# ubc-vision/COTR

Measured on NVIDIA H100. Metric: query-points/sec (256x256 pair, 1024 queries), higher is better.
Workload: dtype f32 (fp16 hi/lo split operands, fp32 accumulate on wgmma)

## Files before the change

cotr_b200/csrc/common.cuh:

```cuda
#pragma once
#include <cuda_fp16.h>
#include <cuda_runtime.h>
#include <cstdarg>
#include <cstdint>
#include <cstdio>

namespace cotr {

void set_error(const char* fmt, ...);

#define COTR_CHECK_CUDA(expr)                                                                      \
    do {                                                                                           \
        cudaError_t e_ = (expr);                                                                   \
        if (e_ != cudaSuccess) {                                                                   \
            ::cotr::set_error("%s:%d: %s -> %s", __FILE__, __LINE__, #expr, cudaGetErrorString(e_)); \
            return 1;                                                                              \
        }                                                                                          \
    } while (0)

#define COTR_CHECK(cond, ...)                                                                      \
    do {                                                                                           \
        if (!(cond)) {                                                                             \
            ::cotr::set_error(__VA_ARGS__);                                                        \
            return 1;                                                                              \
// ... 27 lines not shown
    attr[0].id = cudaLaunchAttributeProgrammaticStreamSerialization;
    attr[0].val.programmaticStreamSerializationAllowed = 1;
    cfg.attrs = attr;
    cfg.numAttrs = g_use_pdl ? 1 : 0;
    return cudaLaunchKernelEx(&cfg, kernel, KArgs(args)...);
}

template <typename... KArgs, typename... Args>
inline cudaError_t launch_kernel_cluster(void (*kernel)(KArgs...), dim3 grid, dim3 block, size_t smem, cudaStream_t s,
                                         int cluster_z, Args... args) {
    cudaLaunchConfig_t cfg = {};
    cfg.gridDim = grid;
    cfg.blockDim = block;
    cfg.dynamicSmemBytes = smem;
    cfg.stream = s;
    cudaLaunchAttribute attr[2];
    int n = 0;
    if (g_use_pdl) {
        attr[n].id = cudaLaunchAttributeProgrammaticStreamSerialization;
        attr[n].val.programmaticStreamSerializationAllowed = 1;
        ++n;
    }
    if (cluster_z > 1) {
        attr[n].id = cudaLaunchAttributeClusterDimension;
        attr[n].val.clusterDim.x = 1;
        attr[n].val.clusterDim.y = 1;
        attr[n].val.clusterDim.z = (unsigned)cluster_z;
        ++n;
    }
    cfg.attrs = attr;
    cfg.numAttrs = n;
    return cudaLaunchKernelEx(&cfg, kernel, KArgs(args)...);
}

constexpr int kNumSms = 132;

constexpr int kDModel = 256;
constexpr int kHeads = 8;
constexpr int kHeadDim = 32;
constexpr int kTokens = 512;
constexpr int kFF = 1024;
constexpr int kEncLayers = 6;
constexpr int kDecLayers = 6;

constexpr size_t kAttnKPlaneBytes = 4 * 512 * 16;
constexpr size_t kAttnKImgBytes = 2 * kAttnKPlaneBytes;
constexpr size_t kAttnVGroupBytes = 2 * 32 * 16 + 16;
constexpr size_t kAttnVImgBytes = 64 * kAttnVGroupBytes;
constexpr size_t kAttnHeadImgBytes = kAttnKImgBytes + kAttnVImgBytes;

struct Split16 {
    __half* hi;
    __half* lo;
};
struct CSplit16 {
    const __half* hi;
    const __half* lo;
};
inline CSplit16 cs(const Split16& s) { return CSplit16{s.hi, s.lo}; }
inline Split16 offset(const Split16& s, size_t elems) { return Split16{s.hi + elems, s.lo + elems}; }
inline CSplit16 offset(const CSplit16& s, size_t elems) { return CSplit16{s.hi + elems, s.lo + elems}; }

constexpr int kStemCanvasRows = 262, kStemCanvasPitch = 264;
constexpr size_t kStemCanvasElems = (size_t)kStemCanvasRows * kStemCanvasPitch * 4;
constexpr int kStemK = 7 * 32;

// ... 122 lines not shown
```

cotr_b200/csrc/gemm_tc.cu:

```cuda
#include <cmath>
#include <cstring>
#include <vector>

#include "a_loader.cuh"
#include "tc_common.cuh"

namespace cotr {

int g_tc_variant = 0;
int g_use_pdl = 1;

namespace {

using namespace tc;

constexpr int BK = 64;
constexpr int kThreads = 384;
constexpr int kConsumerThreads = 256;
constexpr int kBarConsumers = 6;
constexpr long long kWaveCtas = 144;

enum LoaderMode : int { LD_GATHER = 0, LD_CONV = 1, LD_STEM4 = 2 };

__host__ __device__ inline int tc_npad(int N) { return N >= 64 ? ((N + 63) / 64) * 64 : ((N + 15) / 16) * 16; }

template <int BN>
struct Cfg {
    static constexpr int BM = BN >= 256 ? 64 : 128;
    static constexpr int WN = BN >= 256 ? 128 : BN;
    static constexpr uint32_t kAPlane = BM * 128u;
    static constexpr uint32_t kBPlane = BN * 128u;
    static constexpr uint32_t kStage = 2 * kAPlane + 2 * kBPlane;
    static constexpr int kStagesRaw = (int)((227u * 1024u - 3072u) / kStage);
    static constexpr int kStages = kStagesRaw > 4 ? 4 : kStagesRaw;
    static constexpr int kMain = WN >= 128 ? 1 : (WN == 64 ? 2 : 4);
    static constexpr int kCorr = WN >= 64 ? 1 : 2;
    static constexpr int kAccRegs = WN / 2;
    static constexpr uint32_t kAccPitch = BN * 4u + 16u;
    static constexpr uint32_t kAccTileBytes = ((BM * kAccPitch + 1023u) / 1024u) * 1024u;
    static constexpr uint32_t kOutPitch = BN * 2u + 16u;
    static constexpr uint32_t kWarpStaging = 2u * 32u * kOutPitch;
    static constexpr int kChunksN = BN / 16;
    static constexpr int kEpiHalves = (BN >= 32 && BN < 256) ? 2 : 1;
    static constexpr int kChunksW = kChunksN / kEpiHalves;
    static constexpr int kRing = kChunksW < 2 ? kChunksW : 2;
    static constexpr uint32_t kVecOffset = kStages * kStage + 256;
    static constexpr uint32_t kVecBytes = 2u * BN * 4u + 2u * BM * 8u;
    static constexpr uint32_t kSmemBytes = kStages * kStage + 2048 + kVecBytes;
    static constexpr uint32_t kPartOffset = kVecOffset + kVecBytes;
    static constexpr uint32_t kPartPitch = BN * 4u;
    static constexpr int kMaxSplit = BN <= 64 ? 4 : 1;
    static constexpr uint32_t kPartMaxBytes = kMaxSplit > 1 ? 96u * kPartPitch : 0u;
    static_assert(kSmemBytes + kPartMaxBytes <= 227u * 1024u, "split-K partial tiles do not fit");
    static_assert(kStages >= 2, "pipeline needs at least two stages");
    static_assert(kAccTileBytes + (BM / 32) * kWarpStaging <= kStages * kStage, "epilogue tiles do not fit the idle stages");
    static_assert(kStage % 1024 == 0 && kAPlane % 1024 == 0, "stages must stay 1024-byte aligned for SWIZZLE_128B");
    static_assert(kMaxSplit == 1 || BM == 128, "split-K hands over 32-row groups of a 128-row tile");
};

struct EpiOperands {
    float4 bias[4];
    float4 add[4];
    uint4 res_hi[2], res_lo[2];
};

template <int BN, bool LN, int MODE, bool DLN>
__global__ void __launch_bounds__(kThreads, 1) gemm_tc_kernel(const GemmParams p, const int npad) {
    using C = Cfg<BN>;
    constexpr int BM = C::BM;
    extern __shared__ uint8_t smem_raw[];
    const uint32_t raw_addr = smem_u32(smem_raw);
    uint8_t* stage_base = smem_raw + (((raw_addr + 1023u) & ~1023u) - raw_addr);
    uint64_t* bars = reinterpret_cast<uint64_t*>(stage_base + C::kStages * C::kStage);
    uint64_t* full_a = bars;
    uint64_t* empty = bars + C::kStages;
    uint64_t* part_full = bars + 2 * C::kStages;
    uint64_t* vec_full = bars + 2 * C::kStages + 1;
    float* vec_a = reinterpret_cast<float*>(stage_base + C::kVecOffset);
    float* vec_b = vec_a + BN;
    float2* st_a = reinterpret_cast<float2*>(vec_b + BN);
    float2* st_r = st_a + BM;
    float* acc_tile = reinterpret_cast<float*>(stage_base);
    static_assert(!DLN || (MODE == LD_GATHER && !LN), "deferred LayerNorm: row-major operand tiles only");
    constexpr bool kCanLnA = DLN;
    const bool has_aln = kCanLnA && p.a_ln_cs != nullptr;
    const bool stage_vec = kCanLnA && !LN && (has_aln || p.res_ln_part != nullptr);

    const int warp = threadIdx.x >> 5, lane = threadIdx.x & 31;
    const int m0 = blockIdx.x * BM;
    const int n0 = blockIdx.y * BN;
    const int ksplit = gridDim.z;
    const int kz = blockIdx.z;
    const int KC = ((p.K + BK - 1) / BK) / ksplit;
    const int it0 = kz * KC;

    if (threadIdx.x == 0) {
        for (int s = 0; s < C::kStages; ++s) {
            mbar_init(&full_a[s], 129);
            mbar_init(&empty[s], 8);
        }
        mbar_init(part_full, 1);
        if (DLN) mbar_init(vec_full, 64);
        mbar_fence_init();
        if (ksplit > 1) mbar_arrive_expect_tx(part_full, (uint32_t)(ksplit - 1) * (uint32_t)(BM / ksplit) * C::kPartPitch);
    }
    __syncthreads();
    if (ksplit > 1) cluster_arrive();

    if (warp >= 8) {
        const int t = threadIdx.x - kConsumerThreads;
        const int kg = t & 7;
        const int rb = t >> 3;
        constexpr int kRowIters = BM / 16;
        const uint8_t* wimg = reinterpret_cast<const uint8_t*>(p.Wtc);
        auto load_weights = [&](int it) {
            const int s = it % C::kStages;
            mbar_arrive_expect_tx(&full_a[s], 2u * C::kBPlane);
            uint8_t* b_dst = stage_base + (size_t)s * C::kStage + 2 * C::kAPlane;
            const uint8_t* src = wimg + (((size_t)(it0 + it) * 2) * npad + n0) * 128;
            tma_bulk_g2s(b_dst, src, C::kBPlane, &full_a[s]);
            tma_bulk_g2s(b_dst + C::kBPlane, src + (size_t)npad * 128, C::kBPlane, &full_a[s]);
        };
        const int u = (warp - 10) * 32 + lane;
        const float* src_a = has_aln ? p.a_ln_cs : p.res_ln_gamma;
        float va[(BN + 63) / 64], vb[(BN + 63) / 64];
        if (stage_vec && warp >= 10) {
#pragma unroll
            for (int k = 0; k < (BN + 63) / 64; ++k) {
                const int i = u + 64 * k;
                const bool ok = i < BN && n0 + i < p.N;
                va[k] = ok ? __ldg(src_a + n0 + i) : 0.f;
                vb[k] = (ok && !has_aln) ? __ldg(p.res_ln_beta + n0 + i) : 0.f;
            }
        }
        ARow rows[kRowIters];
#pragma unroll
        for (int i = 0; i < kRowIters; ++i) rows[i] = decode_a_row(p, m0 + rb + 16 * i);
        const uint32_t a_off = (uint32_t)rb * 128u + (uint32_t)((kg ^ (rb & 7)) << 4);
        const uint32_t dst0 = smem_u32(stage_base) + a_off;
        if (t == 0) {
            for (int it = 0; it < KC && it < C::kStages; ++it) load_weights(it);
            pdl_launch_dependents();
        }
        pdl_wait();

#pragma unroll 1
        for (int it = 0; it < KC; ++it) {
            const int s = it % C::kStages;
            const uint32_t ph = (uint32_t)(it / C::kStages) & 1u;
            mbar_wait(&empty[s], ph ^ 1u);
            if (t == 0 && it >= C::kStages) load_weights(it);
            const int k0 = (it0 + it) * BK;
            {
                const uint32_t dst = dst0 + (uint32_t)s * C::kStage;
                int kh = 0, kw = 0, koff = k0 + kg * 8;
                if constexpr (MODE == LD_CONV) {
                    const int tap = k0 / p.C;
                    koff = k0 - tap * p.C + kg * 8;
                    kh = tap / p.KW;
                    kw = tap - kh * p.KW;
                }
                if constexpr (MODE == LD_STEM4) {
                    const int kk = k0 + kg * 8;
                    koff = (kk >> 5) * (kStemCanvasPitch * 4) + (kk & 31);
                }
                const bool k_ok = (k0 + kg * 8) < p.K;
#pragma unroll
                for (int i = 0; i < kRowIters; ++i) {
                    bool ok = rows[i].valid && k_ok;
                    size_t off = rows[i].off + koff;
                    if constexpr (MODE == LD_CONV) {
                        const int ih = rows[i].ih0 + kh, iw = rows[i].iw0 + kw;
                        ok = ok && ih >= 0 && ih < p.H && iw >= 0 && iw < p.W;
                        off = rows[i].off + ((size_t)ih * p.W + iw) * p.C + koff;
                    }
                    if (!ok) off = 0;
                    const uint32_t bytes = ok ? 16u : 0u;
                    cp_async16(dst + i * 2048, p.a.hi + off, bytes);
                    cp_async16(dst + C::kAPlane + i * 2048, p.a.lo + off, bytes);
                }
                cp_async_mbar_arrive_noinc(&full_a[s]);
            }
        }

// ... 29 lines not shown
            for (int k = 0; k < (BN + 63) / 64; ++k) {
                const int i = u + 64 * k;
                if (i < BN) { vec_a[i] = va[k]; vec_b[i] = vb[k]; }
            }
            if (has_aln) stage_stats(p.a_ln_part, st_a);
            if (p.res_ln_part != nullptr) stage_stats(p.res_ln_part, st_r);
            mbar_arrive(vec_full);
        }
    } else {
        const int wg = warp >> 2;
        const uint32_t a_sub = BN >= 256 ? 0u : (uint32_t)wg * 64u * 128u;
        const uint32_t b_sub = BN >= 256 ? (uint32_t)wg * 128u * 128u : 0u;
        float acc_m[C::kMain][C::kAccRegs], acc_c[C::kCorr][C::kAccRegs];
#pragma unroll
        for (int a = 0; a < C::kMain; ++a)
#pragma unroll
            for (int j = 0; j < C::kAccRegs; ++j) acc_m[a][j] = 0.f;
#pragma unroll
        for (int a = 0; a < C::kCorr; ++a)
#pragma unroll
            for (int j = 0; j < C::kAccRegs; ++j) acc_c[a][j] = 0.f;
        auto mma = [&](float (&d)[C::kAccRegs], uint64_t da, uint64_t db) {
            if constexpr (C::WN == 16) wgmma_ss_n16(d, da, db);
            else if constexpr (C::WN == 32) wgmma_ss_n32(d, da, db);
            else if constexpr (C::WN == 64) wgmma_ss_n64(d, da, db);
            else wgmma_ss_n128(d, da, db);
        };
        auto fence_all = [&]() {
#pragma unroll
            for (int a = 0; a < C::kMain; ++a) fence_regs(acc_m[a]);
#pragma unroll
            for (int a = 0; a < C::kCorr; ++a) fence_regs(acc_c[a]);
        };
#pragma unroll 1
        for (int it = 0; it < KC; ++it) {
            const int s = it % C::kStages;
            const uint32_t ph = (uint32_t)(it / C::kStages) & 1u;
            mbar_wait(&full_a[s], ph);
            fence_proxy_async_smem();
            const uint32_t a_addr = smem_u32(stage_base + (size_t)s * C::kStage);
            const uint32_t b_addr = a_addr + 2 * C::kAPlane;
            fence_all();
            wgmma_fence();
#pragma unroll
            for (int ks = 0; ks < BK / 16; ++ks) {
                const uint64_t dah = make_desc_sw128(a_addr + a_sub + 32 * ks);
                const uint64_t dal = make_desc_sw128(a_addr + C::kAPlane + a_sub + 32 * ks);
                const uint64_t dbh = make_desc_sw128(b_addr + b_sub + 32 * ks);
                const uint64_t dbl = make_desc_sw128(b_addr + C::kBPlane + b_sub + 32 * ks);
                mma(acc_c[0], dal, dbh);
                mma(acc_m[ks % C::kMain], dah, dbh);
                mma(acc_c[C::kCorr - 1], dah, dbl);
            }
            wgmma_commit();
            wgmma_wait<1>();
            fence_all();
            if (it > 0 && lane == 0) mbar_arrive(&empty[(it - 1) % C::kStages]);
        }
        wgmma_wait<0>();
        fence_all();
        named_barrier_sync(kBarConsumers, kConsumerThreads);
        const int r0 = (BN >= 256 ? 0 : wg * 64) + (warp & 3) * 16 + (lane >> 2);
        const int c0 = (BN >= 256 ? wg * 128 : 0) + 2 * (lane & 3);
#pragma unroll
        for (int j = 0; j < C::kAccRegs; j += 2) {
            float v[2];
#pragma unroll
            for (int e = 0; e < 2; ++e) {
                float x = acc_c[0][j + e];
#pragma unroll
                for (int a = 1; a < C::kCorr; ++a) x += acc_c[a][j + e];
                float y = acc_m[0][j + e];
#pragma unroll
                for (int a = 1; a < C::kMain; ++a) y += acc_m[a][j + e];
                v[e] = x + y;
            }
            const int row = r0 + ((j >> 1) & 1) * 8;
            const int col = c0 + (j >> 2) * 8;
            *reinterpret_cast<float2*>(reinterpret_cast<uint8_t*>(acc_tile) + (uint32_t)row * C::kAccPitch + col * 4) = make_float2(v[0], v[1]);
        }
        named_barrier_sync(kBarConsumers, kConsumerThreads);
    }

    const int ew = warp & 3;
    const int half = warp >> 2;
    if (ksplit > 1) cluster_wait();
    if (warp < 8 && half < C::kEpiHalves && ew * 32 < BM) {
        pdl_wait();
        const int cbeg = half * C::kChunksW * 16;
        const int row = m0 + ew * 32 + lane;
        const int owner = (ew * ksplit) >> 2;
        const bool mine = owner == kz;
        const bool row_ok = mine && row < p.M;
        uint8_t* arow = reinterpret_cast<uint8_t*>(acc_tile) + (uint32_t)(ew * 32 + lane) * C::kAccPitch;
        const float* add_row = (row_ok && p.addmat) ? p.addmat + (size_t)(row % p.add_period) * p.ld_add : nullptr;
        const bool has_res = row_ok && p.res.hi != nullptr;
        const size_t res_off = (size_t)(row_ok ? row : 0) * p.ldr;
        const float acc_scale = p.acc_scale;
        const bool res_ln = kCanLnA && has_res && p.res_ln_part != nullptr;
        float2 res_st = make_float2(0.f, 1.f);
        float res_shift = 0.f;
        float2 a_st = make_float2(0.f, 1.f);
        const bool emit_part = kCanLnA && row_ok && p.ln_part_out != nullptr;
        const bool tail = p.out_f32 != nullptr && (p.N & 15) != 0;
        const bool has_bias = p.bias != nullptr && !tail;

        auto prefetch = [&](int nb, EpiOperands& o) {
            if (nb >= p.N || tail) return;
// ... 53 lines not shown
        constexpr uint32_t kPartPitch = C::kPartPitch, kPartOffset = C::kPartOffset;
        const uint32_t part_slot = (uint32_t)(BM / ksplit) * kPartPitch;
        const uint32_t part_row = (uint32_t)((ew - owner * (4 / ksplit)) * 32 + lane) * kPartPitch;
        const uint32_t part_swz = (uint32_t)(lane & 7);
        auto sum_acc = [&](int c, float (&v)[16]) {
#pragma unroll
            for (int j = 0; j < 16; j += 4) {
                const float4 t4 = *reinterpret_cast<const float4*>(arow + (c + j) * 4);
                v[j] = t4.x; v[j + 1] = t4.y; v[j + 2] = t4.z; v[j + 3] = t4.w;
            }
        };
        auto finish_acc = [&](int c, float (&v)[16]) {
            if (ksplit > 1) {
                const uint8_t* part = stage_base + kPartOffset + part_row;
                for (int peer = 0; peer < ksplit - 1; ++peer) {
#pragma unroll
                    for (int j = 0; j < 16; j += 4) {
                        const uint32_t piece = ((uint32_t)((c + j) >> 2) ^ part_swz) << 4;
                        const float4 t4 = *reinterpret_cast<const float4*>(part + (uint32_t)peer * part_slot + piece);
                        v[j] += t4.x; v[j + 1] += t4.y; v[j + 2] += t4.z; v[j + 3] += t4.w;
                    }
                }
            }
#pragma unroll
            for (int j = 0; j < 16; ++j) v[j] *= acc_scale;
        };
        auto load_acc = [&](int c, float (&v)[16]) {
            sum_acc(c, v);
            finish_acc(c, v);
        };

        size_t tile_base = 0;
        const bool direct = p.out_f32 != nullptr || out_location(p, m0, n0, tile_base);
        uint8_t* const stg_base = stage_base + C::kAccTileBytes;
        uint8_t* stg = stg_base + (uint32_t)ew * C::kWarpStaging + (uint32_t)lane * C::kOutPitch;
        auto emit16 = [&](int c, const float (&v)[16]) {
            if (direct) {
                if (row_ok && n0 + c < p.N) store16(p, row, n0 + c, v);
                return;
            }
            uint4 h0, l0, h1, l1;
            split_f16x2(v[0], v[1], h0.x, l0.x);   split_f16x2(v[2], v[3], h0.y, l0.y);
            split_f16x2(v[4], v[5], h0.z, l0.z);   split_f16x2(v[6], v[7], h0.w, l0.w);
            split_f16x2(v[8], v[9], h1.x, l1.x);   split_f16x2(v[10], v[11], h1.y, l1.y);
            split_f16x2(v[12], v[13], h1.z, l1.z); split_f16x2(v[14], v[15], h1.w, l1.w);
            uint8_t* d = stg + c * 2;
            *reinterpret_cast<uint4*>(d) = h0;
            *reinterpret_cast<uint4*>(d + 16) = h1;
            *reinterpret_cast<uint4*>(d + 32 * C::kOutPitch) = l0;
            *reinterpret_cast<uint4*>(d + 32 * C::kOutPitch + 16) = l1;
        };
        auto drain_plane = [&](int plane) {
            constexpr int kLanesPerRow = BN * 2 / 16;
            constexpr int kRowsPerPass = kLanesPerRow >= 32 ? 1 : 32 / kLanesPerRow;
            constexpr int kPiecesPerLane = kLanesPerRow > 32 ? kLanesPerRow / 32 : 1;
            const uint8_t* wbase = stg_base + (uint32_t)ew * C::kWarpStaging;
            const int r_in = kLanesPerRow >= 32 ? 0 : lane / kLanesPerRow;
            const int piece0 = kLanesPerRow >= 32 ? lane : lane % kLanesPerRow;
            __half* gout = (plane == 0 ? p.out.hi : p.out.lo) + tile_base;
#pragma unroll 4
            for (int r0 = 0; r0 < 32; r0 += kRowsPerPass) {
                const int rr = r0 + r_in;
                const int grow_ = m0 + ew * 32 + rr;
#pragma unroll
                for (int q = 0; q < kPiecesPerLane; ++q) {
                    const int piece = piece0 + q * 32;
                    const uint4 val = *reinterpret_cast<const uint4*>(wbase + (uint32_t)(plane * 32 + rr) * C::kOutPitch + piece * 16);
                    if (grow_ < p.M)
                        *reinterpret_cast<uint4*>(gout + (size_t)(ew * 32 + rr) * p.ldc + piece * 8) = val;
                }
            }
        };
        auto drain = [&]() {
            if (direct) return;
            if constexpr (C::kEpiHalves == 2) {
                named_barrier_sync(1 + ew, 64);
                drain_plane(half);
            } else {
                __syncwarp();
                drain_plane(0);
                drain_plane(1);
            }
        };

        EpiOperands ops[C::kRing];
        const int nbase = (LN ? 0 : n0) + cbeg;
#pragma unroll
        for (int i = 0; i < C::kRing; ++i) prefetch(nbase + 16 * i, ops[i]);
        if (kCanLnA && (has_aln || p.res_ln_part != nullptr)) {
            mbar_wait(vec_full, 0);
            if (has_aln) a_st = st_a[ew * 32 + lane];
            if (res_ln) { res_st = st_r[ew * 32 + lane]; res_shift = -res_st.x * res_st.y; }
        }
        constexpr bool kPreload = !LN && C::kChunksW <= 2;
        float pre[kPreload ? C::kChunksW : 1][16];
        if constexpr (kPreload) {
#pragma unroll
            for (int ci = 0; ci < C::kChunksW; ++ci) sum_acc(cbeg + ci * 16, pre[ci]);
        }
        if (C::kMaxSplit > 1 && ksplit > 1) {
            if (!mine) {
                const uint32_t local = smem_u32(stage_base) + kPartOffset + (uint32_t)(kz < owner ? kz : kz - 1) * part_slot + part_row;
// ... 74 lines not shown
            const float mean = sum * (1.f / 256.f);
            const float dm = mean - shift;
            const float var = fmaxf(sq * (1.f / 256.f) - dm * dm, 0.f);
            const float rstd = 1.f / sqrtf(var + 1e-5f);
#pragma unroll 1
            for (int c = 0; c < BN; c += 32) {
#pragma unroll
                for (int h = 0; h < 2; ++h) {
                    float r[16];
                    sum_acc(c + h * 16, r);
                    float v[16];
#pragma unroll
                    for (int j = 0; j < 16; j += 4) {
                        const float4 g4 = __ldg(reinterpret_cast<const float4*>(p.ln_gamma + c + h * 16 + j));
                        const float4 b4 = __ldg(reinterpret_cast<const float4*>(p.ln_beta + c + h * 16 + j));
                        v[j] = (r[j] - mean) * rstd * g4.x + b4.x;
                        v[j + 1] = (r[j + 1] - mean) * rstd * g4.y + b4.y;
                        v[j + 2] = (r[j + 2] - mean) * rstd * g4.z + b4.z;
                        v[j + 3] = (r[j + 3] - mean) * rstd * g4.w + b4.w;
                    }
                    emit16(c + h * 16, v);
                }
            }
            drain();
        }
        }
    }

    __syncthreads();
}

template <int BN, bool LN, int MODE, bool DLN = false>
int launch_one(const GemmParams& p, cudaStream_t s) {
    using C = Cfg<BN>;
    static unsigned long long configured = 0;
    if (first_use_on_device(&configured)) {
        COTR_CHECK_CUDA(cudaFuncSetAttribute(gemm_tc_kernel<BN, LN, MODE, DLN>, cudaFuncAttributeMaxDynamicSharedMemorySize,
                                             (int)(C::kSmemBytes + C::kPartMaxBytes)));
    }
    const int npad = tc_npad(p.N);
    dim3 grid((p.M + C::BM - 1) / C::BM, (p.N + BN - 1) / BN);
    int ksplit = 1;
    if constexpr (!LN && BN <= 64 && MODE != LD_STEM4) {
        const int kc = (p.K + BK - 1) / BK;
        const long long ctas = (long long)grid.x * grid.y;
        if (!(g_tc_variant & 512) && kc >= (16 >> ((g_tc_variant >> 14) & 3))) {
            if (C::kMaxSplit >= 4 && kc % 4 == 0 && ctas * 4 <= kWaveCtas) ksplit = 4;
            else if (C::kMaxSplit >= 2 && kc % 2 == 0 && ctas * 2 <= kWaveCtas) ksplit = 2;
        }
    }
    COTR_CHECK(p.a_ln_cs == nullptr || (DLN && p.K == 256 && p.a_mode == A_ROWMAJOR && p.a_ln_part != nullptr),
               "gemm_tc: the deferred LayerNorm on A needs a row-major operand with K = 256 and its partial statistics");
    COTR_CHECK((p.res_ln_part == nullptr && p.ln_part_out == nullptr) || DLN,
               "gemm_tc: deferred-LayerNorm residual / statistics on an unsupported tile");
    COTR_CHECK(p.ln_part_out == nullptr || (p.N == 256 && !p.remap && p.out_f32 == nullptr), "gemm_tc: row statistics need a plain N = 256 output");
    grid.z = ksplit;
    const size_t smem = C::kSmemBytes + (size_t)(ksplit - 1) * (C::BM / ksplit) * C::kPartPitch;
    COTR_CHECK_CUDA(launch_kernel_cluster(gemm_tc_kernel<BN, LN, MODE, DLN>, grid, dim3(kThreads), smem, s, ksplit, p, npad));
    return 0;
}

template <int BN, bool LN>
int launch_mode(const GemmParams& p, cudaStream_t s) {
    const bool gather = (p.a_mode == A_ROWMAJOR || p.a_mode == A_TOKENS);
    if (gather && (p.K & 7) == 0 && (p.lda & 7) == 0) {
        if constexpr (!LN) {
            const bool dln = p.a_ln_cs != nullptr || p.res_ln_part != nullptr || p.ln_part_out != nullptr;
            if (dln) return launch_one<BN, LN, LD_GATHER, true>(p, s);
        }
        return launch_one<BN, LN, LD_GATHER>(p, s);
    }
    if constexpr (!LN && BN >= 32) {
        if (p.a_mode == A_CONV_NHWC && (p.C & 63) == 0) return launch_one<BN, LN, LD_CONV>(p, s);
    }
    if constexpr (!LN && BN == 64) {
        if (p.a_mode == A_STEM_NHWC4 && p.K == kStemK) return launch_one<64, false, LD_STEM4>(p, s);
    }
    set_error("gemm_tc: no kernel instantiation for a_mode %d, K %d, lda %d, C %d with tile N %d", p.a_mode, p.K, p.lda, p.C, BN);
    return 1;
}

inline uint16_t f32_to_f16_rn(float f) {
    uint32_t x;
    memcpy(&x, &f, 4);
    const uint16_t sign = (uint16_t)((x >> 16) & 0x8000u);
    x &= 0x7FFFFFFFu;
    if (x >= 0x47800000u) return sign | 0x7BFFu;
    if (x < 0x38800000u) {
        float af;
        memcpy(&af, &x, 4);
        const uint32_t m = (uint32_t)nearbyintf(af * 16777216.0f);
        return sign | (uint16_t)m;
    }
    const uint32_t mant = x & 0x7FFFFFu;
    uint32_t h = (((x >> 23) - 112u) << 10) | (mant >> 13);
    const uint32_t rem = mant & 0x1FFFu;
    if (rem > 0x1000u || (rem == 0x1000u && (h & 1u))) ++h;
    if (h >= 0x7C00u) h = 0x7BFFu;
    return sign | (uint16_t)h;
}
inline float f16_to_f32(uint16_t h) {
    const uint32_t sign = (uint32_t)(h & 0x8000u) << 16;
    const uint32_t e = (h >> 10) & 0x1Fu, m = h & 0x3FFu;
    float mag;
    if (e == 0) mag = (float)m * (1.0f / 16777216.0f);
    else {
// ... 29 lines not shown
    const float scale = ldexpf(1.f, e);
    uint16_t* out = reinterpret_cast<uint16_t*>(dst_host);
    for (int kc = 0; kc < kc_n; ++kc)
        for (int r = 0; r < npad; ++r)
            for (int c = 0; c < 8; ++c)
                for (int el = 0; el < 8; ++el) {
                    const int k = kc * BK + c * 8 + el;
                    const float x = (r < N && k < K) ? w[(size_t)r * K + k] * scale : 0.f;
                    const uint16_t hi = f32_to_f16_rn(x);
                    const uint16_t lo = f32_to_f16_rn(x - f16_to_f32(hi));
                    const size_t pos = (size_t)r * 64 + (size_t)((c ^ (r & 7)) * 8) + el;
                    out[((size_t)kc * 2 + 0) * npad * 64 + pos] = hi;
                    out[((size_t)kc * 2 + 1) * npad * 64 + pos] = lo;
                }
    return ldexpf(1.f, -e);
}

int launch_gemm_tc(const GemmParams& p, cudaStream_t s) {
    COTR_CHECK(p.M > 0 && p.N > 0 && p.K > 0, "gemm_tc: empty problem %d x %d x %d", p.M, p.N, p.K);
    COTR_CHECK(p.Wtc != nullptr, "gemm_tc: weight has no tensor-core image");
    COTR_CHECK(p.out_f32 != nullptr || (p.N & 15) == 0, "gemm_tc: split16 outputs need N %% 16 == 0 (N=%d)", p.N);
    COTR_CHECK(p.res.hi == nullptr || ((p.ldr & 15) == 0 && (p.N & 15) == 0 && ((uintptr_t)p.res.hi & 31) == 0 && ((uintptr_t)p.res.lo & 31) == 0),
               "gemm_tc: residual needs ldr %% 16 == 0 and 32-byte aligned planes");
    COTR_CHECK(p.addmat == nullptr || ((p.ld_add & 3) == 0 && (p.N & 15) == 0), "gemm_tc: add-matrix needs ld %% 4 == 0");
    COTR_CHECK(p.out_f32 != nullptr || (p.ldc & 7) == 0, "gemm_tc: split16 output needs ldc %% 8 == 0");
    if (p.ln_gamma) {
        COTR_CHECK(p.N == 256 && p.relu == 0 && p.out_f32 == nullptr && !p.remap, "gemm_tc: LayerNorm epilogue needs N = 256");
        return launch_mode<256, true>(p, s);
    }
    if (p.N < 64) {
        COTR_CHECK(p.N <= 16, "gemm_tc: N between 17 and 63 is not instantiated");
        return launch_mode<16, false>(p, s);
    }
    const long long mt = (p.M + 127) / 128;
    static const long long kThr[4] = {86, 43, 57, 132};
    const long long thr64 = kThr[(g_tc_variant >> 10) & 3];
    if (mt * ((p.N + 63) / 64) >= thr64 || p.a_mode == A_STEM_NHWC4 || (p.N % 32) != 0) return launch_mode<64, false>(p, s);
    return launch_mode<32, false>(p, s);
}

}
```

cotr_b200/csrc/mlp_tc.cu:

```cuda
#include "split16.cuh"
#include "tc_common.cuh"

namespace cotr {

namespace {

using namespace tc;

constexpr int BM = 64;
constexpr int BK = 64;
constexpr int kThreads = 384;
constexpr int kConsumerThreads = 256;
constexpr int kBarConsumers = 6;
constexpr int kK1Chunks = kDModel / BK;

template <int S>
struct MlpCfg {
    static constexpr int HS = kFF / S;
    static constexpr int WN1 = HS / 2;
    static constexpr int kMain1 = WN1 >= 128 ? 1 : 2;
    static constexpr int kK2Chunks = HS / BK;
    static constexpr int kIters = kK1Chunks + kK2Chunks;
    static constexpr uint32_t kAPlane = BM * 128u;
    static constexpr uint32_t kW1Plane = HS * 128u;
// ... 233 lines not shown
            pdl_wait();
            float v[8];
            const uint8_t* own = base + (uint32_t)rr * C::kAccPitch + lane * 32;
            const float4 a0 = *reinterpret_cast<const float4*>(own), a1 = *reinterpret_cast<const float4*>(own + 16);
            v[0] = a0.x; v[1] = a0.y; v[2] = a0.z; v[3] = a0.w; v[4] = a1.x; v[5] = a1.y; v[6] = a1.z; v[7] = a1.w;
#pragma unroll 1
            for (int slot = 0; slot < S - 1; ++slot) {
                const uint8_t* pp = base + C::kPartOffset + (uint32_t)(slot * C::kOwnRows + w) * C::kRowBytes + lane * 32;
                const float4 b0 = *reinterpret_cast<const float4*>(pp), b1 = *reinterpret_cast<const float4*>(pp + 16);
                v[0] += b0.x; v[1] += b0.y; v[2] += b0.z; v[3] += b0.w; v[4] += b1.x; v[5] += b1.y; v[6] += b1.z; v[7] += b1.w;
            }
            float bias[8], res[8];
            load_vec8(p.b2, lane, bias);
            const size_t off = (size_t)row * kDModel + lane * 8;
            load8_split(p.x, off, res);
#pragma unroll
            for (int j = 0; j < 8; ++j) v[j] = v[j] * p.w2_scale + bias[j] + res[j];
            warp_layernorm256(v, p.g, p.be, lane);
            if (p.g2) warp_layernorm256(v, p.g2, p.be2, lane);
            store8_split(p.out, off, v);
        }
    }
}

template <int S>
int configure(size_t* smem) {
    static unsigned long long configured = 0;
    *smem = MlpCfg<S>::kSmemBytes;
    if (first_use_on_device(&configured))
        COTR_CHECK_CUDA(cudaFuncSetAttribute(mlp_tc_kernel<S>, cudaFuncAttributeMaxDynamicSharedMemorySize, (int)MlpCfg<S>::kSmemBytes));
    return 0;
}

int max_clusters_of_8(int* out) {
    static int cached[64] = {0};
    int dev = 0;
    cudaGetDevice(&dev);
    if (cached[dev & 63] > 0) { *out = cached[dev & 63]; return 0; }
    size_t smem = 0;
    if (configure<8>(&smem)) return 1;
    cudaLaunchConfig_t cfg = {};
    cfg.gridDim = dim3(1, 1, 8);
    cfg.blockDim = dim3(kThreads);
    cfg.dynamicSmemBytes = smem;
    cudaLaunchAttribute attr[1];
    attr[0].id = cudaLaunchAttributeClusterDimension;
    attr[0].val.clusterDim.x = 1;
    attr[0].val.clusterDim.y = 1;
    attr[0].val.clusterDim.z = 8;
    cfg.attrs = attr;
    cfg.numAttrs = 1;
    int n = 0;
    COTR_CHECK_CUDA(cudaOccupancyMaxActiveClusters(&n, mlp_tc_kernel<8>, &cfg));
    cached[dev & 63] = n;
    *out = n;
    return 0;
}

template <int S>
int launch_split(const MlpParams& p, cudaStream_t s) {
    size_t smem = 0;
    if (configure<S>(&smem)) return 1;
    const dim3 grid((p.M + BM - 1) / BM, 1, S);
    COTR_CHECK_CUDA(launch_kernel_cluster(mlp_tc_kernel<S>, grid, dim3(kThreads), smem, s, S, p));
    return 0;
}

}

int launch_mlp_tc(const MlpParams& p, cudaStream_t s) {
    COTR_CHECK(p.M > 0 && p.w1 && p.w2 && p.b1 && p.b2 && p.g && p.be && (p.g2 == nullptr) == (p.be2 == nullptr),
               "mlp_tc: bad parameters (M %d)", p.M);
    const int tiles = (p.M + BM - 1) / BM;
    int n8 = 0;
    if (max_clusters_of_8(&n8)) return 1;
    if (tiles <= n8) return launch_split<8>(p, s);
    return launch_split<4>(p, s);
}

}
```

Before: 1.013 million.

## Pick split-K by cluster occupancy and fold extra K segments in shared memory

Replaces the fixed 144-CTA wave limit for choosing split-K with a query of cudaOccupancyMaxActiveClusters, and factors that query into a shared helper also used by the MLP launcher. For small-N tiles (BN<=32), when a smaller split than the largest divisor is chosen, each CTA now periodically folds its wgmma accumulators into a per-thread shared-memory buffer at segment boundaries. This keeps the per-segment accumulation the same as a full split while using fewer CTAs. It adds extra wgmma_wait<0> drains and shared-memory traffic inside the K loop, and it raises the shared-memory requirement for these tiles.

```diff
diff --git a/cotr_b200/csrc/common.cuh b/cotr_b200/csrc/common.cuh
--- a/cotr_b200/csrc/common.cuh
+++ b/cotr_b200/csrc/common.cuh
@@ -83,6 +83,8 @@
     cfg.numAttrs = n;
     return cudaLaunchKernelEx(&cfg, kernel, KArgs(args)...);
 }
+
+int max_active_clusters(const void* kernel, int threads, size_t smem, int cluster, int* cache, int* out);
 
 constexpr int kNumSms = 132;
 
diff --git a/cotr_b200/csrc/gemm_tc.cu b/cotr_b200/csrc/gemm_tc.cu
--- a/cotr_b200/csrc/gemm_tc.cu
+++ b/cotr_b200/csrc/gemm_tc.cu
@@ -9,6 +9,31 @@
 
 int g_tc_variant = 0;
 int g_use_pdl = 1;
+
+int max_active_clusters(const void* kernel, int threads, size_t smem, int cluster, int* cache, int* out) {
+    int dev = 0;
+    COTR_CHECK_CUDA(cudaGetDevice(&dev));
+    if (cache[dev & 63] > 0) {
+        *out = cache[dev & 63];
+        return 0;
+    }
+    cudaLaunchConfig_t cfg = {};
+    cfg.gridDim = dim3(1, 1, cluster);
+    cfg.blockDim = dim3(threads);
+    cfg.dynamicSmemBytes = smem;
+    cudaLaunchAttribute attr[1];
+    attr[0].id = cudaLaunchAttributeClusterDimension;
+    attr[0].val.clusterDim.x = 1;
+    attr[0].val.clusterDim.y = 1;
+    attr[0].val.clusterDim.z = (unsigned)cluster;
+    cfg.attrs = attr;
+    cfg.numAttrs = 1;
+    int n = 0;
+    COTR_CHECK_CUDA(cudaOccupancyMaxActiveClusters(&n, kernel, &cfg));
+    cache[dev & 63] = n;
+    *out = n;
+    return 0;
+}
 
 namespace {
 
@@ -18,7 +43,6 @@
 constexpr int kThreads = 384;
 constexpr int kConsumerThreads = 256;
 constexpr int kBarConsumers = 6;
-constexpr long long kWaveCtas = 144;
 
 enum LoaderMode : int { LD_GATHER = 0, LD_CONV = 1, LD_STEM4 = 2 };
 
@@ -51,7 +75,10 @@
     static constexpr uint32_t kPartPitch = BN * 4u;
     static constexpr int kMaxSplit = BN <= 64 ? 4 : 1;
     static constexpr uint32_t kPartMaxBytes = kMaxSplit > 1 ? 96u * kPartPitch : 0u;
-    static_assert(kSmemBytes + kPartMaxBytes <= 227u * 1024u, "split-K partial tiles do not fit");
+    static constexpr bool kFold = kMaxSplit > 1 && BN <= 32;
+    static constexpr uint32_t kFoldOffset = kPartOffset + kPartMaxBytes;
+    static constexpr uint32_t kFoldBytes = kFold ? (uint32_t)kConsumerThreads * kAccRegs * 4u : 0u;
+    static_assert(kSmemBytes + kPartMaxBytes + kFoldBytes <= 227u * 1024u, "split-K partial tiles do not fit");
     static_assert(kStages >= 2, "pipeline needs at least two stages");
     static_assert(kAccTileBytes + (BM / 32) * kWarpStaging <= kStages * kStage, "epilogue tiles do not fit the idle stages");
     static_assert(kStage % 1024 == 0 && kAPlane % 1024 == 0, "stages must stay 1024-byte aligned for SWIZZLE_128B");
@@ -65,7 +92,7 @@
 };
 
 template <int BN, bool LN, int MODE, bool DLN>
-__global__ void __launch_bounds__(kThreads, 1) gemm_tc_kernel(const GemmParams p, const int npad) {
+__global__ void __launch_bounds__(kThreads, 1) gemm_tc_kernel(const GemmParams p, const int npad, const int seg) {
     using C = Cfg<BN>;
     constexpr int BM = C::BM;
     extern __shared__ uint8_t smem_raw[];
@@ -245,6 +272,18 @@
 #pragma unroll
             for (int a = 0; a < C::kCorr; ++a) fence_regs(acc_c[a]);
         };
+        auto acc_sum = [&](int j) {
+            float x = acc_c[0][j];
+#pragma unroll
+            for (int a = 1; a < C::kCorr; ++a) x += acc_c[a][j];
+            float y = acc_m[0][j];
+#pragma unroll
+            for (int a = 1; a < C::kMain; ++a) y += acc_m[a][j];
+            return x + y;
+        };
+        float* fold = reinterpret_cast<float*>(stage_base + C::kFoldOffset) + threadIdx.x;
+        const bool folding = C::kFold && seg < KC;
+        int fold_next = seg;
 #pragma unroll 1
         for (int it = 0; it < KC; ++it) {
             const int s = it % C::kStages;
@@ -269,6 +308,27 @@
             wgmma_wait<1>();
             fence_all();
             if (it > 0 && lane == 0) mbar_arrive(&empty[(it - 1) % C::kStages]);
+            if constexpr (C::kFold) {
+                if (folding && it + 1 == fold_next && it + 1 < KC) {
+                    wgmma_wait<0>();
+                    fence_all();
+#pragma unroll
+                    for (int j = 0; j < C::kAccRegs; ++j) {
+                        const float v = acc_sum(j);
+                        fold[j * kConsumerThreads] = it + 1 == seg ? v : fold[j * kConsumerThreads] + v;
+                    }
+#pragma unroll
+                    for (int a = 0; a < C::kMain; ++a)
+#pragma unroll
+                        for (int j = 0; j < C::kAccRegs; ++j) acc_m[a][j] = 0.f;
+#pragma unroll
+                    for (int a = 0; a < C::kCorr; ++a)
+#pragma unroll
+                        for (int j = 0; j < C::kAccRegs; ++j) acc_c[a][j] = 0.f;
+                    fence_all();
+                    fold_next += seg;
+                }
+            }
         }
         wgmma_wait<0>();
         fence_all();
@@ -280,13 +340,8 @@
             float v[2];
 #pragma unroll
             for (int e = 0; e < 2; ++e) {
-                float x = acc_c[0][j + e];
-#pragma unroll
-                for (int a = 1; a < C::kCorr; ++a) x += acc_c[a][j + e];
-                float y = acc_m[0][j + e];
-#pragma unroll
-                for (int a = 1; a < C::kMain; ++a) y += acc_m[a][j + e];
-                v[e] = x + y;
+                v[e] = acc_sum(j + e);
+                if (C::kFold && folding) v[e] = fold[(j + e) * kConsumerThreads] + v[e];
             }
             const int row = r0 + ((j >> 1) & 1) * 8;
             const int col = c0 + (j >> 2) * 8;
@@ -586,27 +641,41 @@
     static unsigned long long configured = 0;
     if (first_use_on_device(&configured)) {
         COTR_CHECK_CUDA(cudaFuncSetAttribute(gemm_tc_kernel<BN, LN, MODE, DLN>, cudaFuncAttributeMaxDynamicSharedMemorySize,
-                                             (int)(C::kSmemBytes + C::kPartMaxBytes)));
+                                             (int)(C::kSmemBytes + C::kPartMaxBytes + C::kFoldBytes)));
     }
     const int npad = tc_npad(p.N);
     dim3 grid((p.M + C::BM - 1) / C::BM, (p.N + BN - 1) / BN);
+    auto smem_of = [](int ks, bool fold) {
+        return fold ? C::kSmemBytes + C::kPartMaxBytes + C::kFoldBytes : C::kSmemBytes + (size_t)(ks - 1) * (C::BM / ks) * C::kPartPitch;
+    };
     int ksplit = 1;
+    int seg = (p.K + BK - 1) / BK;
     if constexpr (!LN && BN <= 64 && MODE != LD_STEM4) {
-        const int kc = (p.K + BK - 1) / BK;
-        const long long ctas = (long long)grid.x * grid.y;
+        const int kc = seg;
+        const int tiles = (int)(grid.x * grid.y);
         if (!(g_tc_variant & 512) && kc >= (16 >> ((g_tc_variant >> 14) & 3))) {
-            if (C::kMaxSplit >= 4 && kc % 4 == 0 && ctas * 4 <= kWaveCtas) ksplit = 4;
-            else if (C::kMaxSplit >= 2 && kc % 2 == 0 && ctas * 2 <= kWaveCtas) ksplit = 2;
-        }
-    }
+            static int fit_cache[C::kMaxSplit + 1][64] = {};
+            int ks_k = 1;
+            for (int ks = C::kMaxSplit; ks >= 2 && ksplit == 1; ks /= 2) {
+                if (kc % ks != 0) continue;
+                if (ks_k == 1) ks_k = ks;
+                int fit = 0;
+                if (max_active_clusters((const void*)gemm_tc_kernel<BN, LN, MODE, DLN>, kThreads, smem_of(ks, C::kFold && ks < C::kMaxSplit),
+                                        ks, fit_cache[ks], &fit)) return 1;
+                if (tiles <= fit) ksplit = ks;
+            }
+            if (C::kFold && ksplit > 1) seg = kc / ks_k;
+        }
+    }
+    const bool fold = seg < (p.K + BK - 1) / BK / ksplit;
     COTR_CHECK(p.a_ln_cs == nullptr || (DLN && p.K == 256 && p.a_mode == A_ROWMAJOR && p.a_ln_part != nullptr),
                "gemm_tc: the deferred LayerNorm on A needs a row-major operand with K = 256 and its partial statistics");
     COTR_CHECK((p.res_ln_part == nullptr && p.ln_part_out == nullptr) || DLN,
                "gemm_tc: deferred-LayerNorm residual / statistics on an unsupported tile");
     COTR_CHECK(p.ln_part_out == nullptr || (p.N == 256 && !p.remap && p.out_f32 == nullptr), "gemm_tc: row statistics need a plain N = 256 output");
     grid.z = ksplit;
-    const size_t smem = C::kSmemBytes + (size_t)(ksplit - 1) * (C::BM / ksplit) * C::kPartPitch;
-    COTR_CHECK_CUDA(launch_kernel_cluster(gemm_tc_kernel<BN, LN, MODE, DLN>, grid, dim3(kThreads), smem, s, ksplit, p, npad));
+    COTR_CHECK_CUDA(launch_kernel_cluster(gemm_tc_kernel<BN, LN, MODE, DLN>, grid, dim3(kThreads), smem_of(ksplit, fold), s, ksplit, p,
+                                          npad, seg));
     return 0;
 }
 
diff --git a/cotr_b200/csrc/mlp_tc.cu b/cotr_b200/csrc/mlp_tc.cu
--- a/cotr_b200/csrc/mlp_tc.cu
+++ b/cotr_b200/csrc/mlp_tc.cu
@@ -289,31 +289,6 @@
     return 0;
 }
 
-int max_clusters_of_8(int* out) {
-    static int cached[64] = {0};
-    int dev = 0;
-    cudaGetDevice(&dev);
-    if (cached[dev & 63] > 0) { *out = cached[dev & 63]; return 0; }
-    size_t smem = 0;
-    if (configure<8>(&smem)) return 1;
-    cudaLaunchConfig_t cfg = {};
-    cfg.gridDim = dim3(1, 1, 8);
-    cfg.blockDim = dim3(kThreads);
-    cfg.dynamicSmemBytes = smem;
-    cudaLaunchAttribute attr[1];
-    attr[0].id = cudaLaunchAttributeClusterDimension;
-    attr[0].val.clusterDim.x = 1;
-    attr[0].val.clusterDim.y = 1;
-    attr[0].val.clusterDim.z = 8;
-    cfg.attrs = attr;
-    cfg.numAttrs = 1;
-    int n = 0;
-    COTR_CHECK_CUDA(cudaOccupancyMaxActiveClusters(&n, mlp_tc_kernel<8>, &cfg));
-    cached[dev & 63] = n;
-    *out = n;
-    return 0;
-}
-
 template <int S>
 int launch_split(const MlpParams& p, cudaStream_t s) {
     size_t smem = 0;
@@ -329,8 +304,11 @@
     COTR_CHECK(p.M > 0 && p.w1 && p.w2 && p.b1 && p.b2 && p.g && p.be && (p.g2 == nullptr) == (p.be2 == nullptr),
                "mlp_tc: bad parameters (M %d)", p.M);
     const int tiles = (p.M + BM - 1) / BM;
+    size_t smem8 = 0;
+    if (configure<8>(&smem8)) return 1;
+    static int n8_cache[64] = {};
     int n8 = 0;
-    if (max_clusters_of_8(&n8)) return 1;
+    if (max_active_clusters((const void*)mlp_tc_kernel<8>, kThreads, smem8, 8, n8_cache, &n8)) return 1;
     if (tiles <= n8) return launch_split<8>(p, s);
     return launch_split<4>(p, s);
 }
```

Result: faster. 1.048 million, median of 6 (+3.4%).

## Add halo-tile loader for 3x3 stride-1 convolutions to reuse input rows across taps

Applied to the files above, without the earlier changes.

Adds an LD_HALO mode for 3x3, stride-1, pad-1 NHWC convolutions. Each CTA loads one padded-pitch halo tile of input channels into shared memory once with cp.async, and the wgmma descriptors are offset per tap instead of re-gathering the A operand for every k-chunk. Output rows are computed on a pitch of W+2, so the epilogue remaps rows and drops the padding columns. This cuts redundant global/L2 loads of the im2col operand at the cost of fewer pipeline stages (100KB reserved for the halo), some wasted MMA rows on padding columns, and a fallback to the old conv path when the halo does not fit or the grid is too small.

```diff
diff --git a/cotr_b200/csrc/gemm_tc.cu b/cotr_b200/csrc/gemm_tc.cu
--- a/cotr_b200/csrc/gemm_tc.cu
+++ b/cotr_b200/csrc/gemm_tc.cu
@@ -20,18 +20,35 @@
 constexpr int kBarConsumers = 6;
 constexpr long long kWaveCtas = 144;
 
-enum LoaderMode : int { LD_GATHER = 0, LD_CONV = 1, LD_STEM4 = 2 };
+enum LoaderMode : int { LD_GATHER = 0, LD_CONV = 1, LD_STEM4 = 2, LD_HALO = 3 };
 
 __host__ __device__ inline int tc_npad(int N) { return N >= 64 ? ((N + 63) / 64) * 64 : ((N + 15) / 16) * 16; }
 
-template <int BN>
+constexpr uint32_t kHaloMaxBytes = 100u * 1024u;
+constexpr int kHaloMaxChunks = 4;
+constexpr long long kHaloMinCtas = 86;
+__host__ __device__ inline int halo_pitch(const GemmParams& p) { return p.W + 2; }
+__host__ __device__ inline int halo_tiles_per_img(const GemmParams& p) { return (p.OH * halo_pitch(p) + 127) / 128; }
+__host__ __device__ inline int halo_rows(const GemmParams& p) { return 128 + 2 * halo_pitch(p) + 2; }
+__host__ __device__ inline uint32_t halo_plane_bytes(const GemmParams& p) { return (uint32_t)((halo_rows(p) + 7) / 8 * 8) * 128u; }
+__device__ __forceinline__ int halo_out_row(const GemmParams& p, int m) {
+    const int tpi = halo_tiles_per_img(p), pitch = halo_pitch(p);
+    const int tile = m >> 7, n = tile / tpi;
+    const int local = (tile - n * tpi) * 128 + (m & 127);
+    const int oh = local / pitch, ow = local - oh * pitch;
+    return (oh < p.OH && ow < p.OW) ? (n * p.OH + oh) * p.OW + ow : -1;
+}
+
+template <int BN, int MODE = LD_GATHER>
 struct Cfg {
     static constexpr int BM = BN >= 256 ? 64 : 128;
     static constexpr int WN = BN >= 256 ? 128 : BN;
     static constexpr uint32_t kAPlane = BM * 128u;
     static constexpr uint32_t kBPlane = BN * 128u;
-    static constexpr uint32_t kStage = 2 * kAPlane + 2 * kBPlane;
-    static constexpr int kStagesRaw = (int)((227u * 1024u - 3072u) / kStage);
+    static constexpr uint32_t kHaloBytes = MODE == LD_HALO ? kHaloMaxBytes : 0u;
+    static constexpr uint32_t kAStage = MODE == LD_HALO ? 0u : 2 * kAPlane;
+    static constexpr uint32_t kStage = kAStage + 2 * kBPlane;
+    static constexpr int kStagesRaw = (int)((227u * 1024u - 3072u - kHaloBytes) / kStage);
     static constexpr int kStages = kStagesRaw > 4 ? 4 : kStagesRaw;
     static constexpr int kMain = WN >= 128 ? 1 : (WN == 64 ? 2 : 4);
     static constexpr int kCorr = WN >= 64 ? 1 : 2;
@@ -46,15 +63,15 @@
     static constexpr int kRing = kChunksW < 2 ? kChunksW : 2;
     static constexpr uint32_t kVecOffset = kStages * kStage + 256;
     static constexpr uint32_t kVecBytes = 2u * BN * 4u + 2u * BM * 8u;
-    static constexpr uint32_t kSmemBytes = kStages * kStage + 2048 + kVecBytes;
+    static constexpr uint32_t kSmemBytes = kHaloBytes + kStages * kStage + 2048 + kVecBytes;
     static constexpr uint32_t kPartOffset = kVecOffset + kVecBytes;
     static constexpr uint32_t kPartPitch = BN * 4u;
     static constexpr int kMaxSplit = BN <= 64 ? 4 : 1;
     static constexpr uint32_t kPartMaxBytes = kMaxSplit > 1 ? 96u * kPartPitch : 0u;
     static_assert(kSmemBytes + kPartMaxBytes <= 227u * 1024u, "split-K partial tiles do not fit");
     static_assert(kStages >= 2, "pipeline needs at least two stages");
-    static_assert(kAccTileBytes + (BM / 32) * kWarpStaging <= kStages * kStage, "epilogue tiles do not fit the idle stages");
-    static_assert(kStage % 1024 == 0 && kAPlane % 1024 == 0, "stages must stay 1024-byte aligned for SWIZZLE_128B");
+    static_assert(kAccTileBytes + (BM / 32) * kWarpStaging <= kHaloBytes + kStages * kStage, "epilogue tiles do not fit the idle stages");
+    static_assert(kStage % 1024 == 0 && kAPlane % 1024 == 0 && kHaloBytes % 1024 == 0, "stages must stay 1024-byte aligned for SWIZZLE_128B");
     static_assert(kMaxSplit == 1 || BM == 128, "split-K hands over 32-row groups of a 128-row tile");
 };
 
@@ -66,21 +83,23 @@
 
 template <int BN, bool LN, int MODE, bool DLN>
 __global__ void __launch_bounds__(kThreads, 1) gemm_tc_kernel(const GemmParams p, const int npad) {
-    using C = Cfg<BN>;
+    using C = Cfg<BN, MODE>;
     constexpr int BM = C::BM;
     extern __shared__ uint8_t smem_raw[];
     const uint32_t raw_addr = smem_u32(smem_raw);
-    uint8_t* stage_base = smem_raw + (((raw_addr + 1023u) & ~1023u) - raw_addr);
+    uint8_t* tile_mem = smem_raw + (((raw_addr + 1023u) & ~1023u) - raw_addr);
+    uint8_t* stage_base = tile_mem + C::kHaloBytes;
     uint64_t* bars = reinterpret_cast<uint64_t*>(stage_base + C::kStages * C::kStage);
     uint64_t* full_a = bars;
     uint64_t* empty = bars + C::kStages;
     uint64_t* part_full = bars + 2 * C::kStages;
     uint64_t* vec_full = bars + 2 * C::kStages + 1;
+    uint64_t* halo_full = bars + 2 * C::kStages + 2;
     float* vec_a = reinterpret_cast<float*>(stage_base + C::kVecOffset);
     float* vec_b = vec_a + BN;
     float2* st_a = reinterpret_cast<float2*>(vec_b + BN);
     float2* st_r = st_a + BM;
-    float* acc_tile = reinterpret_cast<float*>(stage_base);
+    float* acc_tile = reinterpret_cast<float*>(tile_mem);
     static_assert(!DLN || (MODE == LD_GATHER && !LN), "deferred LayerNorm: row-major operand tiles only");
     constexpr bool kCanLnA = DLN;
     const bool has_aln = kCanLnA && p.a_ln_cs != nullptr;
@@ -93,12 +112,23 @@
     const int kz = blockIdx.z;
     const int KC = ((p.K + BK - 1) / BK) / ksplit;
     const int it0 = kz * KC;
+    const int cc = p.C / BK, ccp = cc / ksplit;
+    const uint32_t halo_plane = MODE == LD_HALO ? halo_plane_bytes(p) : 0u;
+    auto w_chunk = [&](int it) {
+        if constexpr (MODE == LD_HALO) {
+            const int tap = it / ccp;
+            return tap * cc + kz * ccp + (it - tap * ccp);
+        }
+        return it0 + it;
+    };
 
     if (threadIdx.x == 0) {
         for (int s = 0; s < C::kStages; ++s) {
-            mbar_init(&full_a[s], 129);
+            mbar_init(&full_a[s], MODE == LD_HALO ? 1 : 129);
             mbar_init(&empty[s], 8);
         }
+        if (MODE == LD_HALO)
+            for (int c = 0; c < ccp; ++c) mbar_init(&halo_full[c], 128);
         mbar_init(part_full, 1);
         if (DLN) mbar_init(vec_full, 64);
         mbar_fence_init();
@@ -116,8 +146,8 @@
         auto load_weights = [&](int it) {
             const int s = it % C::kStages;
             mbar_arrive_expect_tx(&full_a[s], 2u * C::kBPlane);
-            uint8_t* b_dst = stage_base + (size_t)s * C::kStage + 2 * C::kAPlane;
-            const uint8_t* src = wimg + (((size_t)(it0 + it) * 2) * npad + n0) * 128;
+            uint8_t* b_dst = stage_base + (size_t)s * C::kStage + C::kAStage;
+            const uint8_t* src = wimg + (((size_t)w_chunk(it) * 2) * npad + n0) * 128;
             tma_bulk_g2s(b_dst, src, C::kBPlane, &full_a[s]);
             tma_bulk_g2s(b_dst + C::kBPlane, src + (size_t)npad * 128, C::kBPlane, &full_a[s]);
         };
@@ -134,8 +164,10 @@
             }
         }
         ARow rows[kRowIters];
-#pragma unroll
-        for (int i = 0; i < kRowIters; ++i) rows[i] = decode_a_row(p, m0 + rb + 16 * i);
+        if constexpr (MODE != LD_HALO) {
+#pragma unroll
+            for (int i = 0; i < kRowIters; ++i) rows[i] = decode_a_row(p, m0 + rb + 16 * i);
+        }
         const uint32_t a_off = (uint32_t)rb * 128u + (uint32_t)((kg ^ (rb & 7)) << 4);
         const uint32_t dst0 = smem_u32(stage_base) + a_off;
         if (t == 0) {
@@ -143,6 +175,27 @@
             pdl_launch_dependents();
         }
         pdl_wait();
+
+        if constexpr (MODE == LD_HALO) {
+            const int pitch = halo_pitch(p), tpi = halo_tiles_per_img(p), hrows = halo_rows(p);
+            const int n = blockIdx.x / tpi, q0 = (blockIdx.x - n * tpi) * 128;
+            const size_t img = (size_t)n * p.H * p.W * p.C;
+            for (int c = 0; c < ccp; ++c) {
+                const int ch = (kz * ccp + c) * BK + kg * 8;
+                const uint32_t dst = smem_u32(tile_mem) + (uint32_t)c * 2u * halo_plane;
+#pragma unroll 4
+                for (int j = rb; j < hrows; j += 16) {
+                    const int q = q0 + j;
+                    const int ih = q / pitch - 1, iw = q - (ih + 1) * pitch - 1;
+                    const bool ok = ih >= 0 && ih < p.H && iw >= 0 && iw < p.W;
+                    const size_t off = ok ? img + ((size_t)ih * p.W + iw) * p.C + ch : 0;
+                    const uint32_t d = dst + (uint32_t)j * 128u + (uint32_t)((kg ^ (j & 7)) << 4);
+                    cp_async16(d, p.a.hi + off, ok ? 16u : 0u);
+                    cp_async16(d + halo_plane, p.a.lo + off, ok ? 16u : 0u);
+                }
+                cp_async_mbar_arrive_noinc(&halo_full[c]);
+            }
+        }
 
 #pragma unroll 1
         for (int it = 0; it < KC; ++it) {
@@ -150,6 +203,7 @@
             const uint32_t ph = (uint32_t)(it / C::kStages) & 1u;
             mbar_wait(&empty[s], ph ^ 1u);
             if (t == 0 && it >= C::kStages) load_weights(it);
+            if constexpr (MODE == LD_HALO) continue;
             const int k0 = (it0 + it) * BK;
             {
                 const uint32_t dst = dst0 + (uint32_t)s * C::kStage;
@@ -249,16 +303,23 @@
         for (int it = 0; it < KC; ++it) {
             const int s = it % C::kStages;
             const uint32_t ph = (uint32_t)(it / C::kStages) & 1u;
+            uint32_t a_addr = smem_u32(stage_base + (size_t)s * C::kStage);
+            uint32_t a_plane = C::kAPlane;
+            if constexpr (MODE == LD_HALO) {
+                const int tap = it / ccp, c = it - tap * ccp, kh = tap / 3;
+                mbar_wait(&halo_full[c], 0);
+                a_plane = halo_plane;
+                a_addr = smem_u32(tile_mem) + (uint32_t)c * 2u * halo_plane + (uint32_t)(kh * halo_pitch(p) + tap - 3 * kh) * 128u;
+            }
             mbar_wait(&full_a[s], ph);
             fence_proxy_async_smem();
-            const uint32_t a_addr = smem_u32(stage_base + (size_t)s * C::kStage);
-            const uint32_t b_addr = a_addr + 2 * C::kAPlane;
+            const uint32_t b_addr = smem_u32(stage_base + (size_t)s * C::kStage) + C::kAStage;
             fence_all();
             wgmma_fence();
 #pragma unroll
             for (int ks = 0; ks < BK / 16; ++ks) {
                 const uint64_t dah = make_desc_sw128(a_addr + a_sub + 32 * ks);
-                const uint64_t dal = make_desc_sw128(a_addr + C::kAPlane + a_sub + 32 * ks);
+                const uint64_t dal = make_desc_sw128(a_addr + a_plane + a_sub + 32 * ks);
                 const uint64_t dbh = make_desc_sw128(b_addr + b_sub + 32 * ks);
                 const uint64_t dbl = make_desc_sw128(b_addr + C::kBPlane + b_sub + 32 * ks);
                 mma(acc_c[0], dal, dbh);
@@ -406,7 +467,7 @@
 
         size_t tile_base = 0;
         const bool direct = p.out_f32 != nullptr || out_location(p, m0, n0, tile_base);
-        uint8_t* const stg_base = stage_base + C::kAccTileBytes;
+        uint8_t* const stg_base = tile_mem + C::kAccTileBytes;
         uint8_t* stg = stg_base + (uint32_t)ew * C::kWarpStaging + (uint32_t)lane * C::kOutPitch;
         auto emit16 = [&](int c, const float (&v)[16]) {
             if (direct) {
@@ -431,17 +492,23 @@
             const uint8_t* wbase = stg_base + (uint32_t)ew * C::kWarpStaging;
             const int r_in = kLanesPerRow >= 32 ? 0 : lane / kLanesPerRow;
             const int piece0 = kLanesPerRow >= 32 ? lane : lane % kLanesPerRow;
-            __half* gout = (plane == 0 ? p.out.hi : p.out.lo) + tile_base;
+            __half* gout = plane == 0 ? p.out.hi : p.out.lo;
 #pragma unroll 4
             for (int r0 = 0; r0 < 32; r0 += kRowsPerPass) {
                 const int rr = r0 + r_in;
                 const int grow_ = m0 + ew * 32 + rr;
+                bool ok = grow_ < p.M;
+                size_t roff = tile_base + (size_t)(ew * 32 + rr) * p.ldc;
+                if constexpr (MODE == LD_HALO) {
+                    const int orow = halo_out_row(p, grow_);
+                    ok = orow >= 0;
+                    roff = (size_t)orow * p.ldc + n0;
+                }
 #pragma unroll
                 for (int q = 0; q < kPiecesPerLane; ++q) {
                     const int piece = piece0 + q * 32;
                     const uint4 val = *reinterpret_cast<const uint4*>(wbase + (uint32_t)(plane * 32 + rr) * C::kOutPitch + piece * 16);
-                    if (grow_ < p.M)
-                        *reinterpret_cast<uint4*>(gout + (size_t)(ew * 32 + rr) * p.ldc + piece * 8) = val;
+                    if (ok) *reinterpret_cast<uint4*>(gout + roff + piece * 8) = val;
                 }
             }
         };
@@ -582,22 +649,33 @@
 
 template <int BN, bool LN, int MODE, bool DLN = false>
 int launch_one(const GemmParams& p, cudaStream_t s) {
-    using C = Cfg<BN>;
+    using C = Cfg<BN, MODE>;
     static unsigned long long configured = 0;
     if (first_use_on_device(&configured)) {
         COTR_CHECK_CUDA(cudaFuncSetAttribute(gemm_tc_kernel<BN, LN, MODE, DLN>, cudaFuncAttributeMaxDynamicSharedMemorySize,
                                              (int)(C::kSmemBytes + C::kPartMaxBytes)));
     }
     const int npad = tc_npad(p.N);
-    dim3 grid((p.M + C::BM - 1) / C::BM, (p.N + BN - 1) / BN);
+    const int n_img = MODE == LD_HALO ? p.M / (p.OH * p.OW) : 0;
+    dim3 grid(MODE == LD_HALO ? n_img * halo_tiles_per_img(p) : (p.M + C::BM - 1) / C::BM, (p.N + BN - 1) / BN);
     int ksplit = 1;
     if constexpr (!LN && BN <= 64 && MODE != LD_STEM4) {
         const int kc = (p.K + BK - 1) / BK;
+        const int cc = MODE == LD_HALO ? p.C / BK : kc;
         const long long ctas = (long long)grid.x * grid.y;
+        const long long wave = MODE == LD_HALO ? kNumSms : kWaveCtas;
         if (!(g_tc_variant & 512) && kc >= (16 >> ((g_tc_variant >> 14) & 3))) {
-            if (C::kMaxSplit >= 4 && kc % 4 == 0 && ctas * 4 <= kWaveCtas) ksplit = 4;
-            else if (C::kMaxSplit >= 2 && kc % 2 == 0 && ctas * 2 <= kWaveCtas) ksplit = 2;
-        }
+            if (C::kMaxSplit >= 4 && kc % 4 == 0 && cc % 4 == 0 && ctas * 4 <= wave) ksplit = 4;
+            else if (C::kMaxSplit >= 2 && kc % 2 == 0 && cc % 2 == 0 && ctas * 2 <= wave) ksplit = 2;
+        }
+    }
+    if constexpr (MODE == LD_HALO) {
+        const int ccp = p.C / BK / ksplit;
+        if (ccp > kHaloMaxChunks || (uint32_t)ccp * 2u * halo_plane_bytes(p) > kHaloMaxBytes ||
+            (long long)grid.x * grid.y * ksplit < kHaloMinCtas)
+            return launch_one<BN, LN, LD_CONV>(p, s);
+        COTR_CHECK(p.M == n_img * p.OH * p.OW && p.res.hi == nullptr && p.addmat == nullptr && !p.remap && p.out_f32 == nullptr,
+                   "gemm_tc: the halo loader needs whole images and a plain split16 output");
     }
     COTR_CHECK(p.a_ln_cs == nullptr || (DLN && p.K == 256 && p.a_mode == A_ROWMAJOR && p.a_ln_part != nullptr),
                "gemm_tc: the deferred LayerNorm on A needs a row-major operand with K = 256 and its partial statistics");
@@ -610,6 +688,11 @@
     return 0;
 }
 
+inline bool halo_conv(const GemmParams& p) {
+    return p.a_mode == A_CONV_NHWC && p.KH == 3 && p.KW == 3 && p.stride == 1 && p.pad == 1 && p.OH == p.H && p.OW == p.W &&
+           (p.C & 63) == 0 && !(g_tc_variant & (1 << 20));
+}
+
 template <int BN, bool LN>
 int launch_mode(const GemmParams& p, cudaStream_t s) {
     const bool gather = (p.a_mode == A_ROWMAJOR || p.a_mode == A_TOKENS);
@@ -621,7 +704,10 @@
         return launch_one<BN, LN, LD_GATHER>(p, s);
     }
     if constexpr (!LN && BN >= 32) {
-        if (p.a_mode == A_CONV_NHWC && (p.C & 63) == 0) return launch_one<BN, LN, LD_CONV>(p, s);
+        if (p.a_mode == A_CONV_NHWC && (p.C & 63) == 0) {
+            if (halo_conv(p)) return launch_one<BN, LN, LD_HALO>(p, s);
+            return launch_one<BN, LN, LD_CONV>(p, s);
+        }
     }
     if constexpr (!LN && BN == 64) {
         if (p.a_mode == A_STEM_NHWC4 && p.K == kStemK) return launch_one<64, false, LD_STEM4>(p, s);
@@ -717,7 +803,7 @@
         COTR_CHECK(p.N <= 16, "gemm_tc: N between 17 and 63 is not instantiated");
         return launch_mode<16, false>(p, s);
     }
-    const long long mt = (p.M + 127) / 128;
+    const long long mt = halo_conv(p) ? (long long)(p.M / (p.OH * p.OW)) * halo_tiles_per_img(p) : (p.M + 127) / 128;
     static const long long kThr[4] = {86, 43, 57, 132};
     const long long thr64 = kThr[(g_tc_variant >> 10) & 3];
     if (mt * ((p.N + 63) / 64) >= thr64 || p.a_mode == A_STEM_NHWC4 || (p.N % 32) != 0) return launch_mode<64, false>(p, s);
```

Result: faster. 1.016 million before, 1.068 million after (median of 6 runs) (+5.1%).
